# voletiv/mcvd-pytorch

Measured on NVIDIA H100. Metric: frames/sec @100 DDPM steps, SMMNIST 64x64, higher is better.
Workload: dtype f32 (fp16 hi/lo split on wgmma, fp32 accumulate)

## Files before the change

### mcvd_b200/csrc/conv_umma.cu

```cuda
#include <cuda.h>
#include <cuda_fp16.h>

#include <algorithm>
#include <cstring>

#include "mcvd_common.cuh"
#include "umma_ptx.cuh"

namespace mcvd {

constexpr int STAT_MT = 128;

namespace {

using namespace ptx;

constexpr int NPROD = 96;
constexpr int W_LOAD = 3;
constexpr int W_CONS = 4;
constexpr int NT_MAX3 = 192;
constexpr int REG_PROD3 = 96, REG_CONS3 = 136;
constexpr float STAT_SCALE = 65536.0f;
constexpr int TAB_NB = 8;
constexpr int HP_MAX = 512;
constexpr int PPT = (HP_MAX + NPROD - 1) / NPROD;
constexpr int RAW_STAGES = 2;
constexpr int MAX_RESIDENT = 12;

struct ConvMaps {
  CUtensorMap src[4];
  CUtensorMap tab;
};

struct ConvArgs {
  const float* s0;
  const float* s1;
  const float* s2;
  const float* s3;
  int C2, C3, nKB0;
  const __half* wpk;
  const float* bias;
  const float* res;
  const float* tab;
  int tab_planar;
  float* dst;
  unsigned long long* stats;
  int NJ;
  int B, H, W, C0, C1, Cout;
  int ks;
  int Wp, Pimg;
  int Qtot;
  int KB;
  int HP;
  int boxn, nbox;
  int raw_off, raw_stage, tab_off;
  int RA;
  int halo0;
  int nKB;
  int NB;
  int SA;
  int NPI;
  int tiles_n, ntiles;
  int act_in, act_out;
  int split;
  int tab_nb;
  float wscale, oscale;
};

__device__ __forceinline__ int decode_pos(const ConvArgs& a, int q, int& b_out) {
  if (q < 0 || q >= a.Qtot) return -1;
  const int b = q / a.Pimg;
  const int r = q - b * a.Pimg;
  const int rr = r / a.Wp, cc = r - rr * a.Wp;
  b_out = b;
  if (a.ks == 3) {
    if (rr == 0 || cc == 0) return -1;
    return (b * a.H + (rr - 1)) * a.W + (cc - 1);
  }
  return (b * a.H + rr) * a.W + cc;
}

__device__ __forceinline__ int first_raw(const ConvArgs& a, int q) {
  q = max(q, 0);
  if (q >= a.Qtot) return a.B * a.H * a.W;
  if (a.ks == 1) return q;
  const int b = q / a.Pimg;
  const int r = q - b * a.Pimg;
  const int rr = r / a.Wp, cc = r - rr * a.Wp;
  if (rr == 0) return b * a.H * a.W;
  return (b * a.H + (rr - 1)) * a.W + (cc == 0 ? 0 : cc - 1);
}

template <int NT, int NWG>
__global__ void __launch_bounds__(128 * (NWG + 1), 1) k_conv_umma(const ConvArgs a,
                                                                  const __grid_constant__ ConvMaps maps) {
  static_assert(NWG == 2 || (NWG == 3 && NT <= NT_MAX3), "three consumer warpgroups hold at most 96 accumulators");
  constexpr int MT = 64 * NWG;
  constexpr int NTHREADS = 128 * (NWG + 1);
  constexpr int NCONS = 4 * NWG;
  extern __shared__ __align__(1024) uint8_t smem_raw[];
  const int chunks = a.KB / 8;
  const uint32_t a_half_bytes = (uint32_t)chunks * a.HP * 16;
  const uint32_t a_stage_bytes = 2 * a_half_bytes;
  constexpr uint32_t b_step_bytes = 64u * NT;
  const uint32_t b_stage_bytes = (uint32_t)(a.KB / 16) * b_step_bytes;
  uint8_t* a_base = smem_raw;
  uint8_t* b_base = a_base + (size_t)a.SA * a_stage_bytes;
  uint8_t* raw_base = smem_raw + a.raw_off;
  int* pinfo = reinterpret_cast<int*>(raw_base + (size_t)a.RA * a.raw_stage);
  unsigned long long* stat_s = reinterpret_cast<unsigned long long*>(pinfo + PPT * NPROD);
  uint64_t* bars = reinterpret_cast<uint64_t*>(stat_s + (a.stats ? a.NJ * 2 * NT : 0));
  const uint32_t bar0 = smem_u32(bars);
  auto A_FULL = [&](int i) { return bar0 + 8u * i; };
  auto A_EMPTY = [&](int i) { return bar0 + 8u * (a.SA + i); };
  auto B_FULL = [&](int i) { return bar0 + 8u * (2 * a.SA + i); };
  auto B_EMPTY = [&](int i) { return bar0 + 8u * (2 * a.SA + a.NB + i); };
  auto R_FULL = [&](int i) { return bar0 + 8u * (2 * a.SA + 2 * a.NB + i); };
  const int groups_n = a.tiles_n / a.NPI;

  const int tid = threadIdx.x, warp = tid >> 5, lane = tid & 31;
  const int taps = a.ks * a.ks;

  if (tid == 0) {
    for (int i = 0; i < a.SA; ++i) { mbar_init(A_FULL(i), NPROD); mbar_init(A_EMPTY(i), NCONS); }
    for (int i = 0; i < a.NB; ++i) { mbar_init(B_FULL(i), 1); mbar_init(B_EMPTY(i), NCONS); }
    for (int i = 0; i < a.RA; ++i) mbar_init(R_FULL(i), 1);
    fence_barrier_init();
  }
  if (a.stats)
    for (int i = tid; i < a.NJ * 2 * NT; i += NTHREADS) stat_s[i] = 0ull;
  __syncthreads();

  if (warp < W_CONS) {
    if constexpr (NWG == 3) setmaxnreg_dec<REG_PROD3>();
    if (warp < W_LOAD) {
      const bool has_tab = a.tab != nullptr;
      const int ch = (lane >> 3) % chunks;
      const int ppass = NPROD / chunks;
      const int pp = warp * (32 / chunks) + (lane & 7) + 8 * ((lane >> 3) / chunks);
      const uint32_t rowb = (uint32_t)a.KB * 4, smask = a.KB == 32 ? 7u : 3u;
      auto tile_b0_of = [&](int t) {
        const int q_first = (t / groups_n) * MT - a.halo0;
        return q_first <= 0 ? 0 : min(a.B - 1, q_first / a.Pimg);
      };
      const uint32_t raw0 = smem_u32(raw_base);
      const uint32_t main_bytes = (uint32_t)a.nbox * a.boxn * rowb, ctr_bytes = (uint32_t)MT * rowb;
      const uint32_t tab_bytes = (uint32_t)a.tab_nb * a.KB * (a.tab_planar ? 12 : 16);
      int it = blockIdx.x, ikb = 0, ig = 0;
      auto issue_next = [&]() {
        if (it >= a.ntiles) return;
        const int p0 = (it / groups_n) * MT;
        const bool seg2 = ikb >= a.nKB0;
        int si, cc0;
        if (!seg2) {
          const int c0 = ikb * a.KB;
          if (c0 < a.C0) { si = 0; cc0 = c0; } else { si = 1; cc0 = c0 - a.C0; }
        } else {
          const int c0 = (ikb - a.nKB0) * a.KB;
          if (c0 < a.C2) { si = 2; cc0 = c0; } else { si = 3; cc0 = c0 - a.C2; }
        }
        const bool use_tab = has_tab && !seg2;
        const uint32_t dst = raw0 + (uint32_t)(ig % a.RA) * a.raw_stage;
        const uint32_t bar = R_FULL(ig % a.RA);
        mbar_arrive_expect_tx(bar, (seg2 ? ctr_bytes : main_bytes) + (use_tab ? tab_bytes : 0u));
        if (seg2) {
          tma_load_2d(dst, &maps.src[si], cc0, first_raw(a, p0), bar);
        } else {
          const int r0 = first_raw(a, p0 - a.halo0);
          for (int i = 0; i < a.nbox; ++i)
            tma_load_2d(dst + (uint32_t)i * a.boxn * rowb, &maps.src[si], cc0, r0 + i * a.boxn, bar);
        }
        if (use_tab) {
          if (a.tab_planar) tma_load_3d(dst + a.tab_off, &maps.tab, ikb * a.KB, 0, tile_b0_of(it), bar);
          else tma_load_2d(dst + a.tab_off, &maps.tab, 4 * ikb * a.KB, tile_b0_of(it), bar);
        }
        ++ig;
        if (++ikb == a.nKB) { ikb = 0; it += gridDim.x; }
      };
      if (tid == 0)
        for (int i = 0; i < a.RA - 1; ++i) issue_next();
      int g = 0;
      for (int t = blockIdx.x; t < a.ntiles; t += gridDim.x) {
        const int p0 = (t / groups_n) * MT;
        const int tb0 = tile_b0_of(t);
        const int raw_m = first_raw(a, p0 - a.halo0), raw_c = first_raw(a, p0);
        named_bar_sync(1, NPROD);
        for (int h = tid; h < a.HP; h += NPROD) {
          int b = tb0;
          const int pix = decode_pos(a, p0 - a.halo0 + h, b);
          pinfo[h] = pix < 0 ? -1 : ((b - tb0) << 16) | (pix - raw_m);
        }
        for (int kb = 0; kb < a.nKB; ++kb, ++g) {
          const int st = g % a.SA;
          const bool seg2 = kb >= a.nKB0;
          const bool use_tab = has_tab && !seg2;
          const int h_lo = seg2 ? a.halo0 : 0, h_hi = seg2 ? a.halo0 + MT : a.HP;
          const int roff = seg2 ? raw_c - raw_m : 0;
          named_bar_sync(1, NPROD);
          if (tid == 0) issue_next();
          mbar_wait(A_EMPTY(st), ((g / a.SA) & 1) ^ 1);
          const int rs = g % a.RA;
          mbar_wait(R_FULL(rs), (g / a.RA) & 1);
          const uint8_t* raw = raw_base + (size_t)rs * a.raw_stage;
          const float* tsm = reinterpret_cast<const float*>(raw + a.tab_off);
          uint8_t* hi_base = a_base + (size_t)st * a_stage_bytes + (size_t)ch * a.HP * 16;
          uint8_t* lo_base = hi_base + a_half_bytes;
          auto load_raw = [&](int info, float4& r0, float4& r1) {
            r0 = r1 = make_float4(0.f, 0.f, 0.f, 0.f);
            if (info >= 0) {
              const uint32_t off = (uint32_t)((info & 0xffff) - roff) * rowb + 32u * ch;
              const uint32_t sw = ((off >> 7) & smask) << 4;
              r0 = *reinterpret_cast<const float4*>(raw + (off ^ sw));
              r1 = *reinterpret_cast<const float4*>(raw + ((off + 16u) ^ sw));
            }
          };
          float tmean[8], tmul[8], tadd[8];
          int tcur = -1;
          int h = h_lo + pp;
          int info_n = h < h_hi ? pinfo[h] : -1;
          float4 n0, n1;
          load_raw(info_n, n0, n1);
#pragma unroll 1
          for (; h < h_hi; h += ppass) {
            const int info = info_n;
            const float4 c0 = n0, c1 = n1;
            info_n = h + ppass < h_hi ? pinfo[h + ppass] : -1;
            load_raw(info_n, n0, n1);
            uint4 hv = make_uint4(0u, 0u, 0u, 0u), lv = hv;
            if (info >= 0) {
              float v[8] = {c0.x, c0.y, c0.z, c0.w, c1.x, c1.y, c1.z, c1.w};
              if (use_tab) {
                const int bidx = info >> 16;
                if (bidx != tcur) {
                  tcur = bidx;
                  if (a.tab_planar) {
                    const float* tb = tsm + bidx * 3 * a.KB + ch * 8;
#pragma unroll
                    for (int e = 0; e < 8; ++e) { tmean[e] = tb[e]; tmul[e] = tb[a.KB + e]; tadd[e] = tb[2 * a.KB + e]; }
                  } else {
                    const float4* tb = reinterpret_cast<const float4*>(tsm) + bidx * a.KB + ch * 8;
#pragma unroll
                    for (int e = 0; e < 8; ++e) {
                      const float4 tv = tb[e];
                      tmean[e] = tv.x; tmul[e] = tv.y * tv.z; tadd[e] = tv.w;
                    }
                  }
                }
#pragma unroll
                for (int e = 0; e < 8; ++e) v[e] = fmaf(v[e] - tmean[e], tmul[e], tadd[e]);
                if (a.act_in) silu_fast8(v);
              }
              uint32_t hw[4], lw[4];
#pragma unroll
              for (int e = 0; e < 4; ++e) split2(v[2 * e], v[2 * e + 1], hw[e], lw[e]);
              hv = make_uint4(hw[0], hw[1], hw[2], hw[3]);
              lv = make_uint4(lw[0], lw[1], lw[2], lw[3]);
            }
            *reinterpret_cast<uint4*>(hi_base + (size_t)h * 16) = hv;
            *reinterpret_cast<uint4*>(lo_base + (size_t)h * 16) = lv;
          }
          fence_proxy_async();
          mbar_arrive(A_FULL(st));
        }
      }
    } else if (warp == W_LOAD) {
      if (elect_one()) {
        const uint32_t b0 = smem_u32(b_base);
        const int per_tile = a.nKB0 * taps + (a.nKB - a.nKB0);
        int st = 0, ph = 1;
        for (int t = blockIdx.x; t < a.ntiles; t += gridDim.x)
         for (int j = 0; j < a.NPI; ++j) {
          const int nt = (t % groups_n) * a.NPI + j;
          const uint8_t* wsrc = reinterpret_cast<const uint8_t*>(a.wpk) + (size_t)nt * per_tile * b_stage_bytes;
          for (int i = 0; i < per_tile; ++i) {
            mbar_wait(B_EMPTY(st), ph);
            mbar_arrive_expect_tx(B_FULL(st), b_stage_bytes);
            bulk_g2s(b0 + (uint32_t)st * b_stage_bytes, wsrc + (size_t)i * b_stage_bytes, b_stage_bytes, B_FULL(st));
            if (++st == a.NB) { st = 0; ph ^= 1; }
          }
        }
      }
      __syncwarp();
    }
  } else {
    if constexpr (NWG == 3) setmaxnreg_inc<REG_CONS3>();
    const int wg = (warp - W_CONS) >> 2;
    const int wq = (warp - W_CONS) & 3;
    const int ksteps = a.KB / 16;
    const uint32_t a_lbo = (uint32_t)a.HP * 16;
    const uint64_t a_proto = make_desc(0, a_lbo, 128), b_proto = make_desc(0, NT * 16, 128);
    const uint32_t a_half16 = a_half_bytes >> 4, b_lo16 = 2u * NT;
    const uint32_t a0_16 = smem_u32(a_base) >> 4, b0_16 = smem_u32(b_base) >> 4;
    const uint32_t a_stage16 = a_stage_bytes >> 4, b_stage16 = b_stage_bytes >> 4;
    const uint32_t a_lbo16 = a_lbo >> 4;
    int bst = 0, bph = 0, g0 = 0;
    for (int t = blockIdx.x; t < a.ntiles; t += gridDim.x, g0 += a.nKB)
     for (int j = 0; j < a.NPI; ++j) {
      const int p0 = (t / groups_n) * MT;
      const int n0 = ((t % groups_n) * a.NPI + j) * NT;
      const bool last_n = j == a.NPI - 1;
      float acc[NT / 2];
#pragma unroll
      for (int i = 0; i < NT / 2; ++i) acc[i] = 0.f;
      int pend_b = -1, pend_a = -1;
      for (int kb = 0; kb < a.nKB; ++kb) {
        const int g = g0 + kb;
        const int st = g % a.SA;
        mbar_wait(A_FULL(st), (g / a.SA) & 1);
        const uint32_t a_hi16 = a0_16 + (uint32_t)st * a_stage16 + (uint32_t)(a.halo0 + 64 * wg);
        const int ntap = (kb < a.nKB0) ? taps : 1;
        for (int tap = 0; tap < ntap; ++tap) {
          mbar_wait(B_FULL(bst), bph);
          const int shift = (a.ks == 3 && kb < a.nKB0) ? ((tap / 3 - 1) * a.Wp + (tap % 3 - 1)) : 0;
          const uint32_t a_tap16 = a_hi16 + (uint32_t)shift;
          const uint32_t b_tap16 = b0_16 + (uint32_t)bst * b_stage16;
          wgmma_fence();
#pragma unroll 1
          for (int s = 0; s < ksteps; ++s) {
            const uint64_t dbh = desc_add(b_proto, b_tap16 + (uint32_t)s * (b_step_bytes >> 4));
            const uint64_t dbl = desc_add(dbh, b_lo16);
            const uint64_t dah = desc_add(a_proto, a_tap16 + (uint32_t)(2 * s) * a_lbo16);
            const uint64_t dal = desc_add(dah, a_half16);
            wgmma_ss<NT>(acc, dah, dbh, 1);
            if (a.split & 1) wgmma_ss<NT>(acc, dal, dbh, 1);
            if (a.split & 2) wgmma_ss<NT>(acc, dah, dbl, 1);
          }
          wgmma_commit();
          wgmma_wait<1>();
          if (pend_b >= 0 && lane == 0) mbar_arrive(B_EMPTY(pend_b));
          if (pend_a >= 0 && lane == 0) mbar_arrive(A_EMPTY(pend_a));
          pend_b = bst;
          pend_a = (tap == ntap - 1 && last_n) ? st : -1;
          if (++bst == a.NB) { bst = 0; bph ^= 1; }
        }
      }
      wgmma_wait<0>();
#pragma unroll
      for (int i = 0; i < NT / 2; ++i) reg_fence(acc[i]);
      if (lane == 0) { mbar_arrive(B_EMPTY(pend_b)); if (pend_a >= 0) mbar_arrive(A_EMPTY(pend_a)); }

      const int r0 = 64 * wg + 16 * wq + (lane >> 2);
      const int cq = 2 * (lane & 3);
      int pix[2], slot[2];
      const int tile_b0 = min(a.B - 1, p0 / a.Pimg);
#pragma unroll
      for (int i = 0; i < 2; ++i) {
        int b = 0;
        pix[i] = decode_pos(a, p0 + r0 + 8 * i, b);
        slot[i] = pix[i] >= 0 ? b - tile_b0 : -1;
      }
      unsigned jmask = 0;
      if (a.stats) {
#pragma unroll 1
        for (int jj = 0; jj < a.NJ; ++jj)
          if (__ballot_sync(0xffffffffu, slot[0] == jj || slot[1] == jj)) jmask |= 1u << jj;
      }
#pragma unroll
      for (int j = 0; j < NT / 8; ++j) {
        const int n = n0 + 8 * j + cq;
        const float2 bv = a.bias ? __ldg(reinterpret_cast<const float2*>(a.bias + n)) : make_float2(0.f, 0.f);
        float v[2][2];
#pragma unroll
        for (int i = 0; i < 2; ++i) {
          float2 rv = make_float2(0.f, 0.f);
          if (a.res && pix[i] >= 0) rv = __ldg(reinterpret_cast<const float2*>(a.res + (long long)pix[i] * a.Cout + n));
          float x0 = (acc[4 * j + 2 * i] * a.wscale + bv.x + rv.x) * a.oscale;
          float x1 = (acc[4 * j + 2 * i + 1] * a.wscale + bv.y + rv.y) * a.oscale;
          if (a.act_out) { x0 = silu_f(x0); x1 = silu_f(x1); }
          v[i][0] = x0; v[i][1] = x1;
          if (pix[i] >= 0) *reinterpret_cast<float2*>(a.dst + (long long)pix[i] * a.Cout + n) = make_float2(x0, x1);
        }
        if (a.stats) {
#pragma unroll 1
          for (int jj = 0; jj < a.NJ; ++jj) {
            if (!(jmask & (1u << jj))) continue;
#pragma unroll
            for (int e = 0; e < 2; ++e) {
              long long s1 = 0;
              unsigned long long s2 = 0;
#pragma unroll
              for (int i = 0; i < 2; ++i) {
                if (slot[i] == jj) {
                  const int xi = __float2int_rn(v[i][e] * STAT_SCALE);
                  s1 += xi;
                  s2 += (unsigned long long)((long long)xi * (long long)xi);
                }
              }
#pragma unroll
              for (int o = 4; o <= 16; o <<= 1) {
                s1 += __shfl_xor_sync(0xffffffffu, s1, o);
                s2 += __shfl_xor_sync(0xffffffffu, s2, o);
              }
              if (lane < 4) {
                unsigned long long* sp = stat_s + (size_t)jj * 2 * NT + 8 * j + cq + e;
                atomicAdd(sp, (unsigned long long)s1);
                atomicAdd(sp + NT, s2);
              }
            }
          }
        }
      }
      if (a.stats) {
        named_bar_sync(2, 32 * NCONS);
        const int et = tid - W_CONS * 32;
        unsigned long long* gp = a.stats + (size_t)(p0 / MT) * a.NJ * 2 * a.Cout;
        for (int i = et; i < a.NJ * 2 * NT; i += 32 * NCONS) {
          const int jp = i / NT, n = i - jp * NT;
          gp[(size_t)jp * a.Cout + n0 + n] = stat_s[i];
          stat_s[i] = 0ull;
        }
        named_bar_sync(2, 32 * NCONS);
      }
    }
  }
}

__global__ void k_pack_weights(const float* __restrict__ w, __half* __restrict__ out, int taps, int Cin, int Cout,
                               int NT, int KB, float scale, int stage_off, int per_unit) {
  const int ksteps = KB / 16, nKB = Cin / KB, nNT = Cout / NT;
  const long long total = (long long)nNT * nKB * taps * ksteps * 2 * NT * 8;
  for (long long i = (long long)blockIdx.x * blockDim.x + threadIdx.x; i < total;
       i += (long long)gridDim.x * blockDim.x) {
    int e = (int)(i % 8);
    long long t = i / 8;
    int n = (int)(t % NT); t /= NT;
    int j = (int)(t % 2); t /= 2;
    int s = (int)(t % ksteps); t /= ksteps;
    int tap = (int)(t % taps); t /= taps;
    int kb = (int)(t % nKB); t /= nKB;
    int nt = (int)t;
    int c = kb * KB + s * 16 + j * 8 + e;
    float v = w[((long long)tap * Cin + c) * Cout + nt * NT + n] * scale;
    __half h = __float2half_rn(v);
    __half l = __float2half_rn(v - __half2float(h));
    long long step = ((long long)nt * per_unit + stage_off + (long long)kb * taps + tap) * ksteps + s;
    long long base = step * (4LL * NT * 8);
    long long o = (long long)(j * NT + n) * 8 + e;
    out[base + o] = h;
    out[base + 2LL * NT * 8 + o] = l;
  }
}

int pick_kb(int C0, int C1) {
  if (C0 % 32 == 0 && C1 % 32 == 0) return 32;
  if (C0 % 16 == 0 && C1 % 16 == 0) return 16;
  return 0;
}

int conv_kb(int C0, int C1, int C2, int C3) {
  int kb = pick_kb(C0, C1);
  if (C2 + C3 > 0 && pick_kb(C2, C3) < kb) kb = pick_kb(C2, C3);
  return kb;
}

struct Plan {
  int HP, NB, NJ;
  int boxn, nbox, tab_nb;
  int raw_off, raw_stage, tab_off, RA;
  size_t smem;
};

constexpr size_t SMEM_LIMIT = 227 * 1024;

size_t round1024(size_t x) { return (x + 1023) & ~(size_t)1023; }

bool make_plan(int H, int W, int ks, int KB, int NT, bool stats, int SA, int MT, Plan& p) {
  const int Wp = ks == 3 ? W + 1 : W;
  const int Pimg = ks == 3 ? (H + 1) * (W + 1) : H * W;
  const int halo0 = ks == 3 ? Wp + 1 : 0;
  p.HP = (MT + 2 * halo0 + 7) & ~7;
  p.NJ = (MT - 1) / Pimg + 2;
  if (p.HP > HP_MAX) return false;
  p.nbox = p.HP > 256 ? 2 : 1;
  p.boxn = p.nbox == 1 ? p.HP : ((p.HP / 2 + 7) & ~7);
  p.tab_nb = std::min(p.HP / Pimg + 2, TAB_NB);
  p.tab_off = p.nbox * p.boxn * KB * 4;
  p.raw_stage = (int)round1024((size_t)p.tab_off + (size_t)p.tab_nb * KB * 16);
  const size_t a_stage = (size_t)2 * (KB / 8) * p.HP * 16;
  const size_t b_stage = (size_t)(KB / 16) * 64 * NT;
  const size_t stat_bytes = stats ? (size_t)p.NJ * 2 * NT * 8 : 0;
  const size_t pinfo_bytes = (size_t)PPT * NPROD * 4;
  size_t bar_bytes = 0, fixed = 0;
  for (p.RA = RAW_STAGES; p.RA >= 1; --p.RA) {
    bar_bytes = 8 * (2 * SA + 20 + p.RA);
    fixed = round1024(SA * a_stage) + (size_t)p.RA * p.raw_stage + pinfo_bytes + stat_bytes + bar_bytes;
    if (fixed + 2 * b_stage <= SMEM_LIMIT) break;
  }
  if (p.RA == 0) return false;
  p.NB = (int)((SMEM_LIMIT - fixed) / b_stage);
  if (p.NB > 10) p.NB = 10;
  p.raw_off = (int)round1024(SA * a_stage + (size_t)p.NB * b_stage);
  p.smem = (size_t)p.raw_off + (size_t)p.RA * p.raw_stage + pinfo_bytes + stat_bytes + bar_bytes;
  return p.smem <= SMEM_LIMIT;
}

using EncodeTiled = CUresult (*)(CUtensorMap*, CUtensorMapDataType, cuuint32_t, void*, const cuuint64_t*,
                                 const cuuint64_t*, const cuuint32_t*, const cuuint32_t*, CUtensorMapInterleave,
                                 CUtensorMapSwizzle, CUtensorMapL2promotion, CUtensorMapFloatOOBfill);

EncodeTiled encode_tiled() {
  static const EncodeTiled fn = [] {
    void* f = nullptr;
    cudaDriverEntryPointQueryResult q;
    if (cudaGetDriverEntryPoint("cuTensorMapEncodeTiled", &f, cudaEnableDefault, &q) != cudaSuccess ||
        q != cudaDriverEntryPointSuccess)
      f = nullptr;
    return reinterpret_cast<EncodeTiled>(f);
  }();
  return fn;
}

int encode_map(CUtensorMap* m, const float* base, int rank, const cuuint64_t* dims, const cuuint64_t* strides,
               const cuuint32_t* box, CUtensorMapSwizzle swz, const char* name) {
  MCVD_CHECK(((uintptr_t)base & 15) == 0, "%s: TMA source %p is not 16-byte aligned", name, (const void*)base);
  for (int i = 0; i < rank; ++i)
    MCVD_CHECK(box[i] >= 1 && box[i] <= 256, "%s: TMA box dimension %u outside [1, 256]", name, box[i]);
  for (int i = 0; i < rank - 1; ++i)
    MCVD_CHECK(strides[i] % 16 == 0, "%s: TMA stride %llu bytes is not a multiple of 16", name,
               (unsigned long long)strides[i]);
  const EncodeTiled enc = encode_tiled();
  MCVD_CHECK(enc != nullptr, "%s: cuTensorMapEncodeTiled unavailable", name);
  const cuuint32_t estr[3] = {1, 1, 1};
  const CUresult r = enc(m, CU_TENSOR_MAP_DATA_TYPE_FLOAT32, (cuuint32_t)rank, const_cast<float*>(base), dims, strides,
                         box, estr, CU_TENSOR_MAP_INTERLEAVE_NONE, swz, CU_TENSOR_MAP_L2_PROMOTION_L2_128B,
                         CU_TENSOR_MAP_FLOAT_OOB_FILL_NONE);
  MCVD_CHECK(r == CUDA_SUCCESS, "%s: cuTensorMapEncodeTiled failed (%d)", name, (int)r);
  return 0;
}

template <int NT, int NWG>
int launch_nt(const ConvArgs& a, const ConvMaps& m, size_t smem, int grid, cudaStream_t s) {
  cudaError_t e = cudaFuncSetAttribute(k_conv_umma<NT, NWG>, cudaFuncAttributeMaxDynamicSharedMemorySize, (int)smem);
  MCVD_CHECK(e == cudaSuccess, "CONV_UMMA: cudaFuncSetAttribute failed: %s", cudaGetErrorString(e));
  k_conv_umma<NT, NWG><<<grid, 128 * (NWG + 1), smem, s>>>(a, m);
  MCVD_CUDA_LAUNCH_CHECK("conv_umma");
  return 0;
}

template <int NT>
int launch_nt(const ConvArgs& a, const ConvMaps& m, size_t smem, int grid, int nwg, cudaStream_t s) {
  if constexpr (NT <= NT_MAX3)
    if (nwg == 3) return launch_nt<NT, 3>(a, m, smem, grid, s);
  return launch_nt<NT, 2>(a, m, smem, grid, s);
}

int launch_conv(const McvdOp& op, cudaStream_t s, bool planar) {
  const char* name = planar ? "CONV_UMMA2" : "CONV_UMMA";
  MCVD_CHECK(op.src0 && op.w && op.dst && (op.C1 == 0 || op.src1), "%s: null pointer", name);
  MCVD_CHECK(op.i0 == 1 || op.i0 == 3, "%s: kernel size %d unsupported", name, op.i0);
  ConvArgs a;
  a.s0 = (const float*)op.src0; a.s1 = (const float*)op.src1; a.wpk = (const __half*)op.w;
  a.s2 = (const float*)op.src2; a.s3 = (const float*)op.src3; a.C2 = op.src2 ? op.C2 : 0; a.C3 = op.src3 ? op.C3 : 0;
  a.bias = (const float*)op.bias; a.res = (const float*)op.aux0; a.tab = (const float*)op.aux1;
  a.tab_planar = planar ? 1 : 0;
  a.dst = (float*)op.dst;
  a.stats = (unsigned long long*)op.dst2;
  a.B = op.B; a.H = op.H; a.W = op.W; a.C0 = op.C0; a.C1 = op.C1; a.Cout = op.Cout; a.ks = op.i0;
  const int NT = op.i1;
  a.KB = conv_kb(op.C0, op.C1, a.C2, a.C3);
  MCVD_CHECK(a.KB != 0, "%s: input channels (%d,%d | %d,%d) must be multiples of 16", name, op.C0, op.C1, a.C2, a.C3);
  MCVD_CHECK(!planar || op.i2 == 0 || op.i2 == a.KB, "CONV_UMMA2: weights packed for K-block %d, the conv uses %d",
             op.i2, a.KB);
  MCVD_CHECK(NT >= 16 && NT <= 256 && NT % 16 == 0 && op.Cout % NT == 0, "%s: n tile %d invalid for Cout %d", name, NT,
             op.Cout);
  if (a.ks == 3) { a.Wp = op.W + 1; a.Pimg = (op.H + 1) * (op.W + 1); }
  else { a.Wp = op.W; a.Pimg = op.H * op.W; }
  MCVD_CHECK((long long)op.B * a.Pimg < (1LL << 31), "%s: too many pixels", name);
  a.Qtot = op.B * a.Pimg;
  MCVD_CHECK(!a.stats || a.Pimg >= 64, "%s: epilogue statistics need images of >= 64 positions", name);
  a.halo0 = (a.ks == 3) ? a.Wp + 1 : 0;
  a.nKB0 = (op.C0 + op.C1) / a.KB;
  a.nKB = a.nKB0 + (a.C2 + a.C3) / a.KB;
  a.tiles_n = op.Cout / NT;
  const long long tiles128 = (a.Qtot + STAT_MT - 1) / STAT_MT;
  int dev = 0, sms = 132;
  cudaGetDevice(&dev);
  cudaDeviceGetAttribute(&sms, cudaDevAttrMultiProcessorCount, dev);
  const int mode = planar ? 0 : op.i2;
  MCVD_CHECK(mode >= 0 && mode <= 2, "%s: work organisation %d", name, mode);
  Plan p;
  const bool can_stay = a.ks == 1 && a.nKB == a.nKB0 && a.tiles_n > 1 && a.nKB <= MAX_RESIDENT &&
                        make_plan(op.H, op.W, a.ks, a.KB, NT, a.stats != nullptr, a.nKB, STAT_MT, p);
  const bool stay = can_stay && (mode == 2 || (mode == 0 && 2 * tiles128 >= sms));
  const int sa_req = planar ? 0 : op.i5;
  MCVD_CHECK(sa_req == 0 || ((sa_req == 2 || sa_req == 3) && !stay), "%s: %d slab stages", name, sa_req);
  a.SA = stay ? a.nKB : (sa_req ? sa_req : 2);
  a.NPI = stay ? a.tiles_n : 1;
  const int mt_req = planar ? 0 : op.i4;
  MCVD_CHECK(mt_req == 0 || mt_req == 128 || mt_req == 192, "%s: tile height %d", name, mt_req);
  const bool can3 = !planar && NT <= NT_MAX3 && !stay && !a.stats &&
                    make_plan(op.H, op.W, a.ks, a.KB, NT, false, a.SA, 192, p) &&
                    (!a.tab || p.HP / a.Pimg + 2 <= TAB_NB);
  MCVD_CHECK(mt_req != 192 || can3, "%s: 192-position tiles need streaming, NT <= %d, no statistics and %dx%d to fit",
             name, NT_MAX3, op.H, op.W);
  auto last_positions = [&](int mt) {
    const long long items = (a.Qtot + mt - 1) / mt * a.tiles_n;
    return (items + sms - 1) / sms * mt;
  };
  const int MT = mt_req ? mt_req : (can3 && p.NB >= 3 && last_positions(192) <= last_positions(128) ? 192 : 128);
  long long tiles_m = (a.Qtot + MT - 1) / MT;
  if (planar) tiles_m = (tiles_m + 1) & ~1LL;
  MCVD_CHECK(make_plan(op.H, op.W, a.ks, a.KB, NT, a.stats != nullptr, a.SA, MT, p),
             "%s: tile does not fit shared memory (W=%d)", name, op.W);
  a.HP = p.HP; a.NB = p.NB; a.NJ = p.NJ;
  a.boxn = p.boxn; a.nbox = p.nbox; a.raw_off = p.raw_off; a.raw_stage = p.raw_stage; a.tab_off = p.tab_off;
  a.RA = p.RA;
  a.act_in = (op.flags & MCVD_F_ACT_IN) ? 1 : 0;
  a.act_out = (op.flags & MCVD_F_ACT_OUT) ? 1 : 0;
  a.wscale = op.f1; a.oscale = op.f0;
  a.split = (op.i3 >= 1 && op.i3 <= 3) ? op.i3 : (op.i3 == 4 ? 0 : 3);
  {
    const int nb = a.HP / a.Pimg + 2;
    MCVD_CHECK(nb <= TAB_NB || !a.tab, "%s: %dx%d images are too small for the fused-norm path", name, op.H, op.W);
    a.tab_nb = (nb <= TAB_NB) ? nb : 0;
  }
  ConvMaps maps;
  memset(&maps, 0, sizeof(maps));
  {
    const float* srcs[4] = {a.s0, a.s1, a.s2, a.s3};
    const int cs[4] = {a.C0, a.C1, a.C2, a.C3};
    const CUtensorMapSwizzle swz = a.KB == 32 ? CU_TENSOR_MAP_SWIZZLE_128B : CU_TENSOR_MAP_SWIZZLE_64B;
    for (int i = 0; i < 4; ++i) {
      if (!cs[i]) continue;
      MCVD_CHECK(srcs[i] != nullptr, "%s: null source %d", name, i);
      const cuuint64_t dims[2] = {(cuuint64_t)cs[i], (cuuint64_t)op.B * op.H * op.W};
      const cuuint64_t strides[1] = {(cuuint64_t)cs[i] * 4};
      const cuuint32_t box[2] = {(cuuint32_t)a.KB, (cuuint32_t)(i < 2 ? a.boxn : MT)};
      if (encode_map(&maps.src[i], srcs[i], 2, dims, strides, box, swz, name)) return -1;
    }
    if (a.tab) {
      const int Cin = op.C0 + op.C1;
      if (planar) {
        const cuuint64_t dims[3] = {(cuuint64_t)Cin, 3, (cuuint64_t)op.B};
        const cuuint64_t strides[2] = {(cuuint64_t)Cin * 4, (cuuint64_t)Cin * 12};
        const cuuint32_t box[3] = {(cuuint32_t)a.KB, 3, (cuuint32_t)a.tab_nb};
        if (encode_map(&maps.tab, a.tab, 3, dims, strides, box, CU_TENSOR_MAP_SWIZZLE_NONE, name)) return -1;
      } else {
        const cuuint64_t dims[2] = {(cuuint64_t)Cin * 4, (cuuint64_t)op.B};
        const cuuint64_t strides[1] = {(cuuint64_t)Cin * 16};
        const cuuint32_t box[2] = {(cuuint32_t)(4 * a.KB), (cuuint32_t)a.tab_nb};
        if (encode_map(&maps.tab, a.tab, 2, dims, strides, box, CU_TENSOR_MAP_SWIZZLE_NONE, name)) return -1;
      }
    }
  }
  MCVD_CHECK(tiles_m * a.tiles_n < (1LL << 31), "%s: too many tiles", name);
  a.ntiles = (int)(tiles_m * (a.tiles_n / a.NPI));
  const int grid = a.ntiles < sms ? a.ntiles : sms;
  switch (NT) {
#define MCVD_NT_CASE(n) case n: return launch_nt<n>(a, maps, p.smem, grid, MT / 64, s);
    MCVD_NT_CASE(16) MCVD_NT_CASE(32) MCVD_NT_CASE(48) MCVD_NT_CASE(64) MCVD_NT_CASE(80) MCVD_NT_CASE(96)
    MCVD_NT_CASE(112) MCVD_NT_CASE(128) MCVD_NT_CASE(144) MCVD_NT_CASE(160) MCVD_NT_CASE(176) MCVD_NT_CASE(192)
    MCVD_NT_CASE(208) MCVD_NT_CASE(224) MCVD_NT_CASE(240) MCVD_NT_CASE(256)
#undef MCVD_NT_CASE
    default: break;
  }
  MCVD_CHECK(false, "%s: n tile %d", name, NT);
}

long long pack(const float* w_taps, int taps, int Cin, int Cout, int n_tile, int KB, void* out, int scale_log2,
               int stage_off, int per_unit, void* stream) {
  if ((KB != 16 && KB != 32) || Cin % KB || n_tile < 16 || n_tile % 16 || Cout % n_tile) {
    set_error("umma_pack_weights: Cin %d / Cout %d / n_tile %d / KB %d unsupported", Cin, Cout, n_tile, KB);
    return -1;
  }
  const long long bytes = (long long)taps * Cin * Cout * 4;
  if (!out) return bytes;
  if (!w_taps) {
    set_error("umma_pack_weights: null input");
    return -1;
  }
  const float scale = ldexpf(1.0f, scale_log2);
  const long long total = (long long)taps * Cin * Cout;
  long long blocks = (total + 255) / 256;
  if (blocks > 132LL * 16) blocks = 132LL * 16;
  k_pack_weights<<<(unsigned)blocks, 256, 0, (cudaStream_t)stream>>>(w_taps, (__half*)out, taps, Cin, Cout, n_tile, KB,
                                                                      scale, stage_off, per_unit);
  if (cudaGetLastError() != cudaSuccess) {
    set_error("umma_pack_weights: launch failed");
    return -2;
  }
  return bytes;
}

}

int launch_conv_umma(const McvdOp& op, cudaStream_t s) { return launch_conv(op, s, false); }
int launch_conv_umma2(const McvdOp& op, cudaStream_t s) { return launch_conv(op, s, true); }

}

extern "C" int mcvd_umma_kblock(int C0, int C1) { return mcvd::pick_kb(C0, C1); }

extern "C" long long mcvd_umma_pack_weights(const float* w_taps, int taps, int Cin, int Cout, int n_tile, int KB,
                                            void* out, int scale_log2, void* stream) {
  return mcvd::pack(w_taps, taps, Cin, Cout, n_tile, KB, out, scale_log2, 0, KB ? (Cin / KB) * taps : 0, stream);
}

extern "C" int mcvd_umma2_plan(int H, int W, int ks, int C0, int C1, int C2, int C3, int n_tile, int stats) {
  const int kb = mcvd::conv_kb(C0, C1, C2, C3);
  mcvd::Plan p;
  if (!kb || n_tile < 16 || n_tile > 256 || n_tile % 16) return 0;
  return mcvd::make_plan(H, W, ks, kb, n_tile, stats != 0, 2, mcvd::STAT_MT, p) ? kb : 0;
}

extern "C" int mcvd_umma2_plan_info(int H, int W, int ks, int C0, int C1, int C2, int C3, int n_tile, int stats,
                                    int* out) {
  const int kb = mcvd_umma2_plan(H, W, ks, C0, C1, C2, C3, n_tile, stats);
  if (!kb || !out) return -1;
  mcvd::Plan p;
  mcvd::make_plan(H, W, ks, kb, n_tile, stats != 0, 2, mcvd::STAT_MT, p);
  out[0] = kb; out[1] = p.HP; out[2] = 2; out[3] = p.RA; out[4] = p.NB; out[5] = p.NJ; out[6] = 0;
  out[7] = (int)p.smem; out[8] = 1; out[9] = 1;
  return 0;
}

extern "C" long long mcvd_umma2_stats_bytes(int B, int H, int W, int ks, int Cout) {
  const long long pimg = ks == 3 ? (long long)(H + 1) * (W + 1) : (long long)H * W;
  const long long tiles = 2 * ((B * pimg + 2 * mcvd::STAT_MT - 1) / (2 * mcvd::STAT_MT));
  const long long nj = (mcvd::STAT_MT - 1) / pimg + 2;
  return tiles * nj * 2 * Cout * 8;
}

extern "C" long long mcvd_umma2_pack_weights(const float* w_taps, int taps, int Cin, int Cout, int n_tile, int KB,
                                             void* out, int scale_log2, int stage_off, int per_unit, void* stream) {
  return mcvd::pack(w_taps, taps, Cin, Cout, n_tile, KB, out, scale_log2, stage_off, per_unit, stream);
}
```

### mcvd_b200/csrc/umma_ptx.cuh

```cuda
#pragma once
#include <cuda_fp16.h>
#include <stdint.h>

#include "wgmma_ops.cuh"

namespace mcvd {
namespace ptx {

__device__ __forceinline__ uint32_t smem_u32(const void* p) { return (uint32_t)__cvta_generic_to_shared(p); }

__device__ __forceinline__ void mbar_init(uint32_t bar, uint32_t count) {
  asm volatile("mbarrier.init.shared::cta.b64 [%0], %1;" ::"r"(bar), "r"(count) : "memory");
}
__device__ __forceinline__ void mbar_arrive(uint32_t bar) {
  asm volatile("{\n\t.reg .b64 st;\n\tmbarrier.arrive.shared::cta.b64 st, [%0];\n\t}" ::"r"(bar) : "memory");
}
__device__ __forceinline__ void mbar_arrive_expect_tx(uint32_t bar, uint32_t bytes) {
  asm volatile("{\n\t.reg .b64 st;\n\tmbarrier.arrive.expect_tx.shared::cta.b64 st, [%0], %1;\n\t}" ::"r"(bar),
               "r"(bytes)
               : "memory");
}
__device__ __forceinline__ void mbar_wait(uint32_t bar, uint32_t parity) {
  uint32_t done;
  do {
    asm volatile(
        "{\n\t"
        ".reg .pred p;\n\t"
        "mbarrier.try_wait.parity.shared::cta.b64 p, [%1], %2;\n\t"
        "selp.u32 %0, 1, 0, p;\n\t"
        "}"
        : "=r"(done)
        : "r"(bar), "r"(parity)
        : "memory");
  } while (!done);
}
__device__ __forceinline__ void named_bar_sync(int id, int nthreads) {
  asm volatile("bar.sync %0, %1;" ::"r"(id), "r"(nthreads) : "memory");
}
__device__ __forceinline__ void bulk_g2s(uint32_t dst, const void* src, uint32_t bytes, uint32_t bar) {
  asm volatile("cp.async.bulk.shared::cluster.global.mbarrier::complete_tx::bytes [%0], [%1], %2, [%3];" ::"r"(dst),
               "l"(src), "r"(bytes), "r"(bar)
               : "memory");
}
__device__ __forceinline__ void tma_load_2d(uint32_t dst, const void* map, int c0, int c1, uint32_t bar) {
  asm volatile(
      "cp.async.bulk.tensor.2d.shared::cluster.global.tile.mbarrier::complete_tx::bytes [%0], [%1, {%2, %3}], [%4];" ::"r"(
          dst),
      "l"(map), "r"(c0), "r"(c1), "r"(bar)
      : "memory");
}
__device__ __forceinline__ void tma_load_3d(uint32_t dst, const void* map, int c0, int c1, int c2, uint32_t bar) {
  asm volatile(
      "cp.async.bulk.tensor.3d.shared::cluster.global.tile.mbarrier::complete_tx::bytes [%0], [%1, {%2, %3, %4}], [%5];" ::"r"(
          dst),
      "l"(map), "r"(c0), "r"(c1), "r"(c2), "r"(bar)
      : "memory");
}
template <int R>
__device__ __forceinline__ void setmaxnreg_dec() { asm volatile("setmaxnreg.dec.sync.aligned.u32 %0;" ::"n"(R)); }
template <int R>
__device__ __forceinline__ void setmaxnreg_inc() { asm volatile("setmaxnreg.inc.sync.aligned.u32 %0;" ::"n"(R)); }
__device__ __forceinline__ void fence_proxy_async() { asm volatile("fence.proxy.async.shared::cta;" ::: "memory"); }
__device__ __forceinline__ void fence_barrier_init() { asm volatile("fence.mbarrier_init.release.cluster;" ::: "memory"); }

__device__ __forceinline__ void wgmma_fence() { asm volatile("wgmma.fence.sync.aligned;" ::: "memory"); }
__device__ __forceinline__ void wgmma_commit() { asm volatile("wgmma.commit_group.sync.aligned;" ::: "memory"); }
template <int N>
__device__ __forceinline__ void wgmma_wait() {
  asm volatile("wgmma.wait_group.sync.aligned %0;" ::"n"(N) : "memory");
}
__device__ __forceinline__ void reg_fence(float& r) { asm volatile("" : "+f"(r)::"memory"); }

__device__ __forceinline__ uint64_t make_desc(uint32_t saddr, uint32_t lbo_bytes, uint32_t sbo_bytes) {
  uint64_t d = 0;
  d |= (uint64_t)((saddr >> 4) & 0x3FFFu);
  d |= (uint64_t)((lbo_bytes >> 4) & 0x3FFFu) << 16;
  d |= (uint64_t)((sbo_bytes >> 4) & 0x3FFFu) << 32;
  return d;
}
__device__ __forceinline__ uint64_t desc_add(uint64_t d, uint32_t units16) { return d + (uint64_t)units16; }

__device__ __forceinline__ uint32_t pack_half2(__half a, __half b) {
  return (uint32_t)__half_as_ushort(a) | ((uint32_t)__half_as_ushort(b) << 16);
}

__device__ __forceinline__ bool elect_one() {
  uint32_t pred;
  asm volatile(
      "{\n\t"
      ".reg .pred p;\n\t"
      "elect.sync _|p, 0xffffffff;\n\t"
      "selp.u32 %0, 1, 0, p;\n\t"
      "}"
      : "=r"(pred));
  return pred != 0;
}

__device__ __forceinline__ float silu_fast(float x) {
  float e, r;
  asm("ex2.approx.ftz.f32 %0, %1;" : "=f"(e) : "f"(x * -1.4426950408889634f));
  asm("rcp.approx.ftz.f32 %0, %1;" : "=f"(r) : "f"(1.0f + e));
  return x * r;
}
__device__ __forceinline__ void silu_fast8(float v[8]) {
  float t[8];
#pragma unroll
  for (int e = 0; e < 8; ++e) t[e] = v[e] * -1.4426950408889634f;
#pragma unroll
  for (int e = 0; e < 8; ++e) asm volatile("ex2.approx.ftz.f32 %0, %0;" : "+f"(t[e]));
#pragma unroll
  for (int e = 0; e < 8; ++e) t[e] += 1.0f;
#pragma unroll
  for (int e = 0; e < 8; ++e) asm volatile("rcp.approx.ftz.f32 %0, %0;" : "+f"(t[e]));
#pragma unroll
  for (int e = 0; e < 8; ++e) v[e] *= t[e];
}
__device__ __forceinline__ void split2(float a, float b, uint32_t& hi, uint32_t& lo) {
  asm("cvt.rn.satfinite.f16x2.f32 %0, %1, %2;" : "=r"(hi) : "f"(b), "f"(a));
  const float2 hf = __half22float2(*reinterpret_cast<const __half2*>(&hi));
  asm("cvt.rn.satfinite.f16x2.f32 %0, %1, %2;" : "=r"(lo) : "f"(b - hf.y), "f"(a - hf.x));
}

}
}
```

Before: 138.9.

## Stage 1x1 conv epilogue through swizzled shared memory and store with TMA

Result: faster. 141.1, median of 6 (+1.6%).

```diff
diff --git a/mcvd_b200/csrc/conv_umma.cu b/mcvd_b200/csrc/conv_umma.cu
--- a/mcvd_b200/csrc/conv_umma.cu
+++ b/mcvd_b200/csrc/conv_umma.cu
@@ -26,10 +26,14 @@
 constexpr int PPT = (HP_MAX + NPROD - 1) / NPROD;
 constexpr int RAW_STAGES = 2;
 constexpr int MAX_RESIDENT = 12;
+constexpr int OUT_COLS = 16;
+constexpr int OUT_STAGES = 2;
+constexpr int OUT_BOX = 64 * OUT_COLS * 4;
 
 struct ConvMaps {
   CUtensorMap src[4];
   CUtensorMap tab;
+  CUtensorMap out;
 };
 
 struct ConvArgs {
@@ -91,10 +95,11 @@
   return (b * a.H + (rr - 1)) * a.W + (cc == 0 ? 0 : cc - 1);
 }
 
-template <int NT, int NWG>
+template <int NT, int NWG, bool TOUT>
 __global__ void __launch_bounds__(128 * (NWG + 1), 1) k_conv_umma(const ConvArgs a,
                                                                   const __grid_constant__ ConvMaps maps) {
   static_assert(NWG == 2 || (NWG == 3 && NT <= NT_MAX3), "three consumer warpgroups hold at most 96 accumulators");
+  static_assert(!TOUT || (NWG == 2 && NT <= NT_MAX3), "the staged epilogue runs on two consumer warpgroups, NT <= 192");
   constexpr int MT = 64 * NWG;
   constexpr int NTHREADS = 128 * (NWG + 1);
   constexpr int NCONS = 4 * NWG;
@@ -107,7 +112,8 @@
   uint8_t* a_base = smem_raw;
   uint8_t* b_base = a_base + (size_t)a.SA * a_stage_bytes;
   uint8_t* raw_base = smem_raw + a.raw_off;
-  int* pinfo = reinterpret_cast<int*>(raw_base + (size_t)a.RA * a.raw_stage);
+  uint8_t* out_base = raw_base + (size_t)a.RA * a.raw_stage;
+  int* pinfo = reinterpret_cast<int*>(out_base + (TOUT ? (size_t)NWG * OUT_STAGES * OUT_BOX : 0));
   unsigned long long* stat_s = reinterpret_cast<unsigned long long*>(pinfo + PPT * NPROD);
   uint64_t* bars = reinterpret_cast<uint64_t*>(stat_s + (a.stats ? a.NJ * 2 * NT : 0));
   const uint32_t bar0 = smem_u32(bars);
@@ -294,6 +300,7 @@
     const uint32_t a_stage16 = a_stage_bytes >> 4, b_stage16 = b_stage_bytes >> 4;
     const uint32_t a_lbo16 = a_lbo >> 4;
     int bst = 0, bph = 0, g0 = 0;
+    int ost = 0;
     for (int t = blockIdx.x; t < a.ntiles; t += gridDim.x, g0 += a.nKB)
      for (int j = 0; j < a.NPI; ++j) {
       const int p0 = (t / groups_n) * MT;
@@ -341,6 +348,58 @@
 
       const int r0 = 64 * wg + 16 * wq + (lane >> 2);
       const int cq = 2 * (lane & 3);
+      if constexpr (TOUT) {
+        const bool leader = wq == 0 && lane == 0;
+        const int rl = r0 - 64 * wg;
+        uint8_t* ostage = out_base + (size_t)wg * OUT_STAGES * OUT_BOX;
+        auto load_res = [&](int c, float2 (&r)[2][2]) {
+#pragma unroll
+          for (int jj = 0; jj < 2; ++jj)
+#pragma unroll
+            for (int i = 0; i < 2; ++i) {
+              const int q = p0 + r0 + 8 * i;
+              r[jj][i] = make_float2(0.f, 0.f);
+              if (a.res && q < a.Qtot)
+                r[jj][i] = __ldg(reinterpret_cast<const float2*>(a.res + (long long)q * a.Cout + n0 + 16 * c + 8 * jj + cq));
+            }
+        };
+        float2 rnext[2][2];
+        load_res(0, rnext);
+#pragma unroll
+        for (int c = 0; c < NT / OUT_COLS; ++c) {
+          float2 rv[2][2];
+#pragma unroll
+          for (int jj = 0; jj < 2; ++jj) { rv[jj][0] = rnext[jj][0]; rv[jj][1] = rnext[jj][1]; }
+          if (c + 1 < NT / OUT_COLS) load_res(c + 1, rnext);
+          uint8_t* box = ostage + ost * OUT_BOX;
+          if (++ost == OUT_STAGES) ost = 0;
+          if (leader) bulk_wait_read<OUT_STAGES - 1>();
+          named_bar_sync(3 + wg, 128);
+#pragma unroll
+          for (int jj = 0; jj < 2; ++jj) {
+            const int j = 2 * c + jj;
+            const int n = n0 + 8 * j + cq;
+            const float2 bv = a.bias ? __ldg(reinterpret_cast<const float2*>(a.bias + n)) : make_float2(0.f, 0.f);
+#pragma unroll
+            for (int i = 0; i < 2; ++i) {
+              const int row = rl + 8 * i;
+              float x0 = (acc[4 * j + 2 * i] * a.wscale + bv.x + rv[jj][i].x) * a.oscale;
+              float x1 = (acc[4 * j + 2 * i + 1] * a.wscale + bv.y + rv[jj][i].y) * a.oscale;
+              if (a.act_out) { x0 = silu_f(x0); x1 = silu_f(x1); }
+              const int col = 8 * jj + cq;
+              const uint32_t off = (uint32_t)row * 64u + ((uint32_t)((col >> 2) ^ ((row >> 1) & 3)) << 4) + (col & 3) * 4u;
+              *reinterpret_cast<float2*>(box + off) = make_float2(x0, x1);
+            }
+          }
+          fence_proxy_async();
+          named_bar_sync(3 + wg, 128);
+          if (leader) {
+            tma_store_2d(&maps.out, smem_u32(box), n0 + OUT_COLS * c, p0 + 64 * wg);
+            bulk_commit();
+          }
+        }
+        continue;
+      }
       int pix[2], slot[2];
       const int tile_b0 = min(a.B - 1, p0 / a.Pimg);
 #pragma unroll
@@ -412,6 +471,7 @@
         named_bar_sync(2, 32 * NCONS);
       }
     }
+    if (TOUT && ((warp - W_CONS) & 3) == 0 && lane == 0) bulk_wait_all();
   }
 }
 
@@ -464,7 +524,7 @@
 
 size_t round1024(size_t x) { return (x + 1023) & ~(size_t)1023; }
 
-bool make_plan(int H, int W, int ks, int KB, int NT, bool stats, int SA, int MT, Plan& p) {
+bool make_plan(int H, int W, int ks, int KB, int NT, bool stats, int SA, int MT, bool tma_out, Plan& p) {
   const int Wp = ks == 3 ? W + 1 : W;
   const int Pimg = ks == 3 ? (H + 1) * (W + 1) : H * W;
   const int halo0 = ks == 3 ? Wp + 1 : 0;
@@ -480,17 +540,18 @@
   const size_t b_stage = (size_t)(KB / 16) * 64 * NT;
   const size_t stat_bytes = stats ? (size_t)p.NJ * 2 * NT * 8 : 0;
   const size_t pinfo_bytes = (size_t)PPT * NPROD * 4;
+  const size_t out_bytes = tma_out ? (size_t)(MT / 64) * OUT_STAGES * OUT_BOX : 0;
   size_t bar_bytes = 0, fixed = 0;
   for (p.RA = RAW_STAGES; p.RA >= 1; --p.RA) {
     bar_bytes = 8 * (2 * SA + 20 + p.RA);
-    fixed = round1024(SA * a_stage) + (size_t)p.RA * p.raw_stage + pinfo_bytes + stat_bytes + bar_bytes;
+    fixed = round1024(SA * a_stage) + (size_t)p.RA * p.raw_stage + out_bytes + pinfo_bytes + stat_bytes + bar_bytes;
     if (fixed + 2 * b_stage <= SMEM_LIMIT) break;
   }
   if (p.RA == 0) return false;
   p.NB = (int)((SMEM_LIMIT - fixed) / b_stage);
   if (p.NB > 10) p.NB = 10;
   p.raw_off = (int)round1024(SA * a_stage + (size_t)p.NB * b_stage);
-  p.smem = (size_t)p.raw_off + (size_t)p.RA * p.raw_stage + pinfo_bytes + stat_bytes + bar_bytes;
+  p.smem = (size_t)p.raw_off + (size_t)p.RA * p.raw_stage + out_bytes + pinfo_bytes + stat_bytes + bar_bytes;
   return p.smem <= SMEM_LIMIT;
 }
 
@@ -528,20 +589,23 @@
   return 0;
 }
 
-template <int NT, int NWG>
+template <int NT, int NWG, bool TOUT>
 int launch_nt(const ConvArgs& a, const ConvMaps& m, size_t smem, int grid, cudaStream_t s) {
-  cudaError_t e = cudaFuncSetAttribute(k_conv_umma<NT, NWG>, cudaFuncAttributeMaxDynamicSharedMemorySize, (int)smem);
+  cudaError_t e = cudaFuncSetAttribute(k_conv_umma<NT, NWG, TOUT>, cudaFuncAttributeMaxDynamicSharedMemorySize,
+                                       (int)smem);
   MCVD_CHECK(e == cudaSuccess, "CONV_UMMA: cudaFuncSetAttribute failed: %s", cudaGetErrorString(e));
-  k_conv_umma<NT, NWG><<<grid, 128 * (NWG + 1), smem, s>>>(a, m);
+  k_conv_umma<NT, NWG, TOUT><<<grid, 128 * (NWG + 1), smem, s>>>(a, m);
   MCVD_CUDA_LAUNCH_CHECK("conv_umma");
   return 0;
 }
 
 template <int NT>
-int launch_nt(const ConvArgs& a, const ConvMaps& m, size_t smem, int grid, int nwg, cudaStream_t s) {
-  if constexpr (NT <= NT_MAX3)
-    if (nwg == 3) return launch_nt<NT, 3>(a, m, smem, grid, s);
-  return launch_nt<NT, 2>(a, m, smem, grid, s);
+int launch_nt(const ConvArgs& a, const ConvMaps& m, size_t smem, int grid, int nwg, bool tout, cudaStream_t s) {
+  if constexpr (NT <= NT_MAX3) {
+    if (nwg == 3) return launch_nt<NT, 3, false>(a, m, smem, grid, s);
+    if (tout) return launch_nt<NT, 2, true>(a, m, smem, grid, s);
+  }
+  return launch_nt<NT, 2, false>(a, m, smem, grid, s);
 }
 
 int launch_conv(const McvdOp& op, cudaStream_t s, bool planar) {
@@ -576,11 +640,12 @@
   int dev = 0, sms = 132;
   cudaGetDevice(&dev);
   cudaDeviceGetAttribute(&sms, cudaDevAttrMultiProcessorCount, dev);
+  const bool out128 = a.ks == 1 && !a.stats && NT <= NT_MAX3;
   const int mode = planar ? 0 : op.i2;
   MCVD_CHECK(mode >= 0 && mode <= 2, "%s: work organisation %d", name, mode);
   Plan p;
   const bool can_stay = a.ks == 1 && a.nKB == a.nKB0 && a.tiles_n > 1 && a.nKB <= MAX_RESIDENT &&
-                        make_plan(op.H, op.W, a.ks, a.KB, NT, a.stats != nullptr, a.nKB, STAT_MT, p);
+                        make_plan(op.H, op.W, a.ks, a.KB, NT, a.stats != nullptr, a.nKB, STAT_MT, out128, p);
   const bool stay = can_stay && (mode == 2 || (mode == 0 && 2 * tiles128 >= sms));
   const int sa_req = planar ? 0 : op.i5;
   MCVD_CHECK(sa_req == 0 || ((sa_req == 2 || sa_req == 3) && !stay), "%s: %d slab stages", name, sa_req);
@@ -589,7 +654,7 @@
   const int mt_req = planar ? 0 : op.i4;
   MCVD_CHECK(mt_req == 0 || mt_req == 128 || mt_req == 192, "%s: tile height %d", name, mt_req);
   const bool can3 = !planar && NT <= NT_MAX3 && !stay && !a.stats &&
-                    make_plan(op.H, op.W, a.ks, a.KB, NT, false, a.SA, 192, p) &&
+                    make_plan(op.H, op.W, a.ks, a.KB, NT, false, a.SA, 192, false, p) &&
                     (!a.tab || p.HP / a.Pimg + 2 <= TAB_NB);
   MCVD_CHECK(mt_req != 192 || can3, "%s: 192-position tiles need streaming, NT <= %d, no statistics and %dx%d to fit",
              name, NT_MAX3, op.H, op.W);
@@ -598,9 +663,10 @@
     return (items + sms - 1) / sms * mt;
   };
   const int MT = mt_req ? mt_req : (can3 && p.NB >= 3 && last_positions(192) <= last_positions(128) ? 192 : 128);
+  const bool tma_out = out128 && MT == 128;
   long long tiles_m = (a.Qtot + MT - 1) / MT;
   if (planar) tiles_m = (tiles_m + 1) & ~1LL;
-  MCVD_CHECK(make_plan(op.H, op.W, a.ks, a.KB, NT, a.stats != nullptr, a.SA, MT, p),
+  MCVD_CHECK(make_plan(op.H, op.W, a.ks, a.KB, NT, a.stats != nullptr, a.SA, MT, tma_out, p),
              "%s: tile does not fit shared memory (W=%d)", name, op.W);
   a.HP = p.HP; a.NB = p.NB; a.NJ = p.NJ;
   a.boxn = p.boxn; a.nbox = p.nbox; a.raw_off = p.raw_off; a.raw_stage = p.raw_stage; a.tab_off = p.tab_off;
@@ -643,11 +709,17 @@
       }
     }
   }
+  if (tma_out) {
+    const cuuint64_t dims[2] = {(cuuint64_t)op.Cout, (cuuint64_t)op.B * op.H * op.W};
+    const cuuint64_t strides[1] = {(cuuint64_t)op.Cout * 4};
+    const cuuint32_t box[2] = {(cuuint32_t)OUT_COLS, 64};
+    if (encode_map(&maps.out, a.dst, 2, dims, strides, box, CU_TENSOR_MAP_SWIZZLE_64B, name)) return -1;
+  }
   MCVD_CHECK(tiles_m * a.tiles_n < (1LL << 31), "%s: too many tiles", name);
   a.ntiles = (int)(tiles_m * (a.tiles_n / a.NPI));
   const int grid = a.ntiles < sms ? a.ntiles : sms;
   switch (NT) {
-#define MCVD_NT_CASE(n) case n: return launch_nt<n>(a, maps, p.smem, grid, MT / 64, s);
+#define MCVD_NT_CASE(n) case n: return launch_nt<n>(a, maps, p.smem, grid, MT / 64, tma_out, s);
     MCVD_NT_CASE(16) MCVD_NT_CASE(32) MCVD_NT_CASE(48) MCVD_NT_CASE(64) MCVD_NT_CASE(80) MCVD_NT_CASE(96)
     MCVD_NT_CASE(112) MCVD_NT_CASE(128) MCVD_NT_CASE(144) MCVD_NT_CASE(160) MCVD_NT_CASE(176) MCVD_NT_CASE(192)
     MCVD_NT_CASE(208) MCVD_NT_CASE(224) MCVD_NT_CASE(240) MCVD_NT_CASE(256)
@@ -700,7 +772,7 @@
   const int kb = mcvd::conv_kb(C0, C1, C2, C3);
   mcvd::Plan p;
   if (!kb || n_tile < 16 || n_tile > 256 || n_tile % 16) return 0;
-  return mcvd::make_plan(H, W, ks, kb, n_tile, stats != 0, 2, mcvd::STAT_MT, p) ? kb : 0;
+  return mcvd::make_plan(H, W, ks, kb, n_tile, stats != 0, 2, mcvd::STAT_MT, false, p) ? kb : 0;
 }
 
 extern "C" int mcvd_umma2_plan_info(int H, int W, int ks, int C0, int C1, int C2, int C3, int n_tile, int stats,
@@ -708,7 +780,7 @@
   const int kb = mcvd_umma2_plan(H, W, ks, C0, C1, C2, C3, n_tile, stats);
   if (!kb || !out) return -1;
   mcvd::Plan p;
-  mcvd::make_plan(H, W, ks, kb, n_tile, stats != 0, 2, mcvd::STAT_MT, p);
+  mcvd::make_plan(H, W, ks, kb, n_tile, stats != 0, 2, mcvd::STAT_MT, false, p);
   out[0] = kb; out[1] = p.HP; out[2] = 2; out[3] = p.RA; out[4] = p.NB; out[5] = p.NJ; out[6] = 0;
   out[7] = (int)p.smem; out[8] = 1; out[9] = 1;
   return 0;
diff --git a/mcvd_b200/csrc/umma_ptx.cuh b/mcvd_b200/csrc/umma_ptx.cuh
--- a/mcvd_b200/csrc/umma_ptx.cuh
+++ b/mcvd_b200/csrc/umma_ptx.cuh
@@ -56,6 +56,17 @@
       "l"(map), "r"(c0), "r"(c1), "r"(c2), "r"(bar)
       : "memory");
 }
+__device__ __forceinline__ void tma_store_2d(const void* map, uint32_t src, int c0, int c1) {
+  asm volatile("cp.async.bulk.tensor.2d.global.shared::cta.bulk_group [%0, {%2, %3}], [%1];" ::"l"(map), "r"(src),
+               "r"(c0), "r"(c1)
+               : "memory");
+}
+__device__ __forceinline__ void bulk_commit() { asm volatile("cp.async.bulk.commit_group;" ::: "memory"); }
+template <int N>
+__device__ __forceinline__ void bulk_wait_read() {
+  asm volatile("cp.async.bulk.wait_group.read %0;" ::"n"(N) : "memory");
+}
+__device__ __forceinline__ void bulk_wait_all() { asm volatile("cp.async.bulk.wait_group 0;" ::: "memory"); }
 template <int R>
 __device__ __forceinline__ void setmaxnreg_dec() { asm volatile("setmaxnreg.dec.sync.aligned.u32 %0;" ::"n"(R)); }
 template <int R>
```
